# sethdford/csm-mlx

Hardware: AMD Instinct MI355X
Metric: audio frames/sec (24 kHz) csm_1b greedy, 10 s utterances, 1/2/4/8 GPU (higher is better)
Workload: dtype bf16; 1 GPU; csm_1b greedy generate(), 10 s utterances (125 frames) + Mimi decode; top_k=0, stream=False, context_segments=0, model=csm_1b (synthetic seed-0 weights), global_batch=1, per_gpu_batch=1, frames=125, mimi_decode=True, parallelism=dp1

## Files before the change

csm-mlx_amd/csrc/dec_frame.hip:

```cpp
#include <type_traits>

#include "c0_process.h"
#include "csm_kernels.h"
#include "handoff.h"
#include "sampler.h"

namespace {

using namespace handoff;

constexpr int NWG = 256, NT = 512;
constexpr int D = 1024, F = 8192, HQ = 8, HKV = 2, HD = 128, NL = DEC_FRAME_LAYERS, DB = 2048;
constexpr int QKV = (HQ + 2 * HKV) * HD;
constexpr int MAXM = 2;
constexpr int VMAX = 2056;

__device__ __forceinline__ void dot8x2(const u32x4_t w, const float* x0, const float* x1, float& s0, float& s1) {
  const float4 a0 = *reinterpret_cast<const float4*>(x0), b0 = *reinterpret_cast<const float4*>(x0 + 4);
  const float4 a1 = *reinterpret_cast<const float4*>(x1), b1 = *reinterpret_cast<const float4*>(x1 + 4);
  float t;
  t = bf16_lo(w.x); s0 = fmaf(t, a0.x, s0); s1 = fmaf(t, a1.x, s1);
  t = bf16_hi(w.x); s0 = fmaf(t, a0.y, s0); s1 = fmaf(t, a1.y, s1);
  t = bf16_lo(w.y); s0 = fmaf(t, a0.z, s0); s1 = fmaf(t, a1.z, s1);
  t = bf16_hi(w.y); s0 = fmaf(t, a0.w, s0); s1 = fmaf(t, a1.w, s1);
  t = bf16_lo(w.z); s0 = fmaf(t, b0.x, s0); s1 = fmaf(t, b1.x, s1);
  t = bf16_hi(w.z); s0 = fmaf(t, b0.y, s0); s1 = fmaf(t, b1.y, s1);
  t = bf16_lo(w.w); s0 = fmaf(t, b0.z, s0); s1 = fmaf(t, b1.z, s1);
  t = bf16_hi(w.w); s0 = fmaf(t, b0.w, s0); s1 = fmaf(t, b1.w, s1);
}

template <int M>
__device__ __forceinline__ void dotm(const u32x4_t w, const float* x0, const float* x1, float& s0, float& s1) {
  if constexpr (M == 2) {
    dot8x2(w, x0, x1, s0, s1);
  } else {
    const float4 a0 = *reinterpret_cast<const float4*>(x0), b0 = *reinterpret_cast<const float4*>(x0 + 4);
    s0 = fmaf(bf16_lo(w.x), a0.x, s0);
    s0 = fmaf(bf16_hi(w.x), a0.y, s0);
    s0 = fmaf(bf16_lo(w.y), a0.z, s0);
    s0 = fmaf(bf16_hi(w.y), a0.w, s0);
    s0 = fmaf(bf16_lo(w.z), b0.x, s0);
    s0 = fmaf(bf16_hi(w.z), b0.y, s0);
    s0 = fmaf(bf16_lo(w.w), b0.z, s0);
    s0 = fmaf(bf16_hi(w.w), b0.w, s0);
  }
}

__device__ __forceinline__ u32x4_t wload(const bf16_t* p) { return *reinterpret_cast<const u32x4_t*>(p); }

struct Lds {
  float x[MAXM][D];
  float xn[MAXM][DB];
  float qkv[MAXM][QKV];
  float att[MAXM][D];
  float qs[HQ][HD];
  float2 rope[MAXM][HD / 2];
  alignas(16) float hb[MAXM][32];
  float red[4 * MAXM][256];
  float wsum[8][MAXM * 8];
  float sq[8][MAXM];
  union {
    float Ks[HKV][32][HD + 4];
    struct {
      float hq[DB / 32][36];
      float hh[DB / 32];
    } h0;
  };
  float Vs[HKV][32][HD];
  float lg[VMAX];
  int flag;
  alignas(16) float xq[MAXM][D / 32][36];
  float xh[MAXM][D / 32];
  alignas(16) float aq[MAXM][D / 32][36];
  float ah[MAXM][D / 32];
  int c0win[C0_WINDOW_MAX];
  float c0b[16];
};

}

namespace {

constexpr int REP = 4;
constexpr size_t G_X = 0;
constexpr size_t G_QKV = G_X + 2 * REP * rs_of(MAXM * D);
constexpr size_t G_PART = G_QKV + 2 * REP * rs_of(MAXM * QKV);
constexpr size_t G_ARG = G_PART + (size_t)2 * NWG * MAXM * D;
constexpr size_t G_LOG = G_ARG + 2 * REP * rs_of(NWG * 2);
constexpr size_t G_GUM = G_LOG + 2 * REP * rs_of(VMAX);
constexpr size_t G_TOTAL = G_GUM + 2 * REP * rs_of(NWG * 3);

struct Ctx : HandoffCtx<DecFrameArgs, Lds, REP> {
  int ps = 0;
  int code = 0;
  __device__ void mark() {
    if (p.stamps && tid == 0 && ps < 496) p.stamps[(size_t)w * DEC_FRAME_STAMPS + 512 + ps] = __builtin_amdgcn_s_memrealtime();
    ++ps;
  }
  __device__ void stamp() const {
    if (p.stamps && tid == 0 && e < DEC_FRAME_STAMPS) p.stamps[(size_t)w * DEC_FRAME_STAMPS + e] = __builtin_amdgcn_s_memrealtime();
  }
};

constexpr int PROBE_DELAY = 16;
constexpr int DELAY_E1 = PROBE_DELAY, DELAY_E3 = PROBE_DELAY, DELAY_E4 = PROBE_DELAY, DELAY_E5 = 40, DELAY_E6 = PROBE_DELAY;
constexpr int REPOLL = 2;

template <int GPT, int DELAY = PROBE_DELAY, typename F>
__device__ __forceinline__ void poll(Ctx& c, const u64* base, const int (&off)[GPT], const bool (&val)[GPT], F&& use) {
  poll_granules<GPT, DELAY, REPOLL>(base, off, val, c.tag(), [&](unsigned spin) { return spin_fail(c, spin); }, use);
  c.stamp();
}

template <int GPT>
__device__ __forceinline__ void gather(Ctx& c, const u64* buf, int n, float* out) {
  int off[GPT];
  bool val[GPT];
#pragma unroll
  for (int u = 0; u < GPT; ++u) {
    off[u] = c.tid + u * NT;
    val[u] = off[u] < n;
  }
  poll<GPT>(c, buf, off, val, [&](const u64 (&g)[GPT]) {
#pragma unroll
    for (int u = 0; u < GPT; ++u)
      if (val[u]) out[off[u]] = __uint_as_float((unsigned)g[u]);
  });
  __syncthreads();
}

__device__ __forceinline__ float2 nw_fetch(const Ctx& c, const float* nw) { return make_float2(nw[2 * c.tid], nw[2 * c.tid + 1]); }

template <int M>
__device__ __forceinline__ void rms_rows(Ctx& c, float2 nw) {
  static_assert(D == 2 * NT, "a thread scales elements 2 tid and 2 tid + 1 of each row");
  if (c.wave < M) {
    const float* x = c.L.x[c.wave];
    float s = 0.f;
    for (int k = c.lane; k < D; k += 64) s = fmaf(x[k], x[k], s);
    s = wave_sum(s);
    if (c.lane == 0) c.L.wsum[0][c.wave] = s;
  }
  __syncthreads();
  for (int m = 0; m < M; ++m) {
    const float r = rsqrtf(c.L.wsum[0][m] / (float)D + c.p.eps);
    c.L.xn[m][2 * c.tid] = c.L.x[m][2 * c.tid] * r * nw.x;
    c.L.xn[m][2 * c.tid + 1] = c.L.x[m][2 * c.tid + 1] * r * nw.y;
  }
  __syncthreads();
}

template <int M, int DELAY>
__device__ __forceinline__ void gather_x(Ctx& c, const u64* buf, float2 nw) {
  static_assert(D == 2 * NT, "pair tid of row m is elements 2 tid, 2 tid + 1");
  float sq[MAXM];
  int poff[M];
#pragma unroll
  for (int m = 0; m < M; ++m) poff[m] = m * D + 2 * c.tid;
  poll_pairs<M, DELAY, REPOLL>(buf, 0x7fffffff, poff, c.tag(), [&](unsigned spin) { return spin_fail(c, spin); },
                               [&](const u32x4_t (&g)[M]) {
#pragma unroll
    for (int m = 0; m < M; ++m) {
      const float v0 = __uint_as_float(g[m].x), v1 = __uint_as_float(g[m].z);
      *reinterpret_cast<float2*>(&c.L.x[m][2 * c.tid]) = make_float2(v0, v1);
      *reinterpret_cast<float2*>(&c.L.xn[m][2 * c.tid]) = make_float2(v0 * nw.x, v1 * nw.y);
      sq[m] = fmaf(v1, v1, v0 * v0);
    }
  });
  c.stamp();
#pragma unroll
  for (int m = 0; m < M; ++m) {
    const float t = wave_sum(sq[m]);
    if (c.lane == 0) c.L.sq[c.wave][m] = t;
  }
  __syncthreads();
}
__device__ __forceinline__ float row_rs(const Ctx& c, int m) {
  float s = c.L.sq[0][m];
#pragma unroll
  for (int w = 1; w < 8; ++w) s += c.L.sq[w][m];
  return rsqrtf(s / (float)D + c.p.eps);
}

struct WQkv { u32x4_t a, b; };
struct WO { u32x4_t a; };
constexpr int GU_EARLY = 4;
struct WGu { u32x4_t a[8][2]; };
struct WDn { u32x4_t a[2][2][2]; };
struct WHd { u32x4_t a[2]; u32x4_t x[2]; };

__device__ __forceinline__ void load_qkv(Ctx& c, int l, WQkv& r) {
  if (c.wave < 6) {
    const bf16_t* row = c.p.wqkv[l] + (size_t)(6 * c.w) * D;
    const int v = (c.wave * D + 8 * c.lane) * 2;
    r.a = bload(row, v, 0);
    r.b = bload(row, v, 1024);
  }
}
__device__ __forceinline__ void load_o(Ctx& c, int l, WO& r) {
  const bf16_t* row = c.p.wo[l] + (size_t)(4 * c.w) * D;
  r.a = bload(row, ((c.wave >> 1) * D + 8 * ((c.wave & 1) * 64 + c.lane)) * 2, 0);
}
template <int I0, int I1>
__device__ __forceinline__ void load_gu(Ctx& c, int l, WGu& r) {
  const bf16_t* base = c.p.wgu[l] + (size_t)(64 * c.w) * D;
  const int v = (8 * c.wave * D + 8 * c.lane) * 2;
#pragma unroll
  for (int i = I0; i < I1; ++i) {
    r.a[i][0] = bload(base, v, i * D * 2);
    r.a[i][1] = bload(base, v, i * D * 2 + 1024);
  }
}
__device__ __forceinline__ void load_dn(Ctx& c, int l, WDn& r) {
  const bf16_t* base = c.p.wdc[l] + (size_t)(2 * c.w) * D * 16;
  const int v = c.tid * 16 * 2 * 2;
#pragma unroll
  for (int s = 0; s < 2; ++s)
#pragma unroll
    for (int q = 0; q < 2; ++q) {
      const int so = (q * D * 16 + s * 16) * 2;
      r.a[s][q][0] = bload(base, v, so);
      r.a[s][q][1] = bload(base, v, so + 16);
    }
}
__device__ __forceinline__ void load_head(Ctx& c, const bf16_t* W, int K, WHd& r) {
  const bf16_t* base = W + (size_t)(8 * c.w) * K;
  const int v = (c.wave * K + 8 * c.lane) * 2;
  r.a[0] = bload<2>(base, v, 0);
  r.a[1] = bload<2>(base, v, 1024);
  if (c.wave == 0 && c.w < 3) {
    const bf16_t* xr = W + (size_t)(2048 + c.w) * K;
    r.x[0] = bload<2>(xr, 16 * c.lane, 0);
    r.x[1] = bload<2>(xr, 16 * c.lane, 1024);
  }
}

constexpr int RB = D / 2, SBR = D / 64 * 4;
constexpr int RBH = DB / 2, SBRH = DB / 64 * 4;
constexpr int SB_QKV = QKV * RB, SB_O = D * RB, SB_GU = 2 * F * RB, SB_DN = D * F / 2, SB_PROJ = D * RBH;
struct WQkv4 { u32x4_t a; unsigned s; };
struct WO4 { u32x4_t a; unsigned s; };
struct WGu4 { u32x4_t a[4]; unsigned s[4]; };
struct WDn4 { u32x4_t a[2]; unsigned s[2]; };
__device__ __forceinline__ int hrow(const Ctx& c) { return c.lane >> 5; }
__device__ __forceinline__ int hgi(const Ctx& c) { return c.lane & 31; }

__device__ __forceinline__ void load_qkv4(Ctx& c, int l, WQkv4& r) {
  if (c.wave < 3) {
    const char* W = reinterpret_cast<const char*>(c.p.wqkv[l]);
    const int row = 2 * c.wave + hrow(c);
    r.a = bload(W, row * RB + hgi(c) * 16, 6 * c.w * RB);
    r.s = bload4(W, row * SBR + (hgi(c) >> 1) * 4, SB_QKV + 6 * c.w * SBR);
  }
}
__device__ __forceinline__ void load_o4(Ctx& c, int l, WO4& r) {
  if (c.wave < 2) {
    const char* W = reinterpret_cast<const char*>(c.p.wo[l]);
    const int row = 2 * c.wave + hrow(c);
    r.a = bload(W, row * RB + hgi(c) * 16, 4 * c.w * RB);
    r.s = bload4(W, row * SBR + (hgi(c) >> 1) * 4, SB_O + 4 * c.w * SBR);
  }
}
template <int I0, int I1>
__device__ __forceinline__ void load_gu4(Ctx& c, int l, WGu4& r) {
  const char* W = reinterpret_cast<const char*>(c.p.wgu[l]);
  const int row = 8 * c.wave + hrow(c);
#pragma unroll
  for (int i = I0; i < I1; ++i) {
    r.a[i] = bload(W, row * RB + hgi(c) * 16, (64 * c.w + 2 * i) * RB);
    r.s[i] = bload4(W, row * SBR + (hgi(c) >> 1) * 4, SB_GU + (64 * c.w + 2 * i) * SBR);
  }
}
__device__ __forceinline__ void load_dn4(Ctx& c, int l, WDn4& r) {
  const char* W = reinterpret_cast<const char*>(c.p.wdc[l]);
#pragma unroll
  for (int k = 0; k < 2; ++k) {
    r.a[k] = bload(W, (2 * c.tid + k) * 16, c.w * D * 16);
    r.s[k] = bload4(W, (2 * c.tid + k) * 4, SB_DN + (c.w >> 1) * D * 4);
  }
}

__device__ __forceinline__ void half_group_sum16(const Ctx& c, float v, float* out) {
  v = sum16(v);
  if ((c.tid & 15) == 0) out[c.tid >> 4] = v;
}

template <int M, bool SC>
__device__ __forceinline__ void qkv_publish(Ctx& c, int pos0);
template <int M, bool SC>
__device__ __forceinline__ void phase_qkv(Ctx& c, int pos0, const WQkv& W) {
  if (c.wave < 6) {
    float s0 = 0.f, s1 = 0.f;
    dotm<M>(W.a, c.L.xn[0] + 8 * c.lane, c.L.xn[1] + 8 * c.lane, s0, s1);
    dotm<M>(W.b, c.L.xn[0] + 8 * (c.lane + 64), c.L.xn[1] + 8 * (c.lane + 64), s0, s1);
    s0 = wave_sum(s0);
    if constexpr (M == 2) s1 = wave_sum(s1);
    if (c.lane == 0) { c.L.wsum[c.wave][0] = s0; if constexpr (M == 2) c.L.wsum[c.wave][1] = s1; }
  }
  __syncthreads();
  qkv_publish<M, SC>(c, pos0);
}
template <int M, bool SC>
__device__ __forceinline__ void phase_qkv4(Ctx& c, int pos0, const WQkv4& W) {
  if (c.wave < 3) {
#pragma unroll
    for (int m = 0; m < M; ++m) {
      const float2 h = half_sums(q4dot32(W.a, c.L.xq[m][hgi(c)], W.s, c.L.xh[m][hgi(c)]));
      if (c.lane == 0) { c.L.wsum[2 * c.wave][m] = h.x; c.L.wsum[2 * c.wave + 1][m] = h.y; }
    }
  }
  __syncthreads();
  qkv_publish<M, SC>(c, pos0);
}
template <int M, bool SC>
__device__ __forceinline__ void qkv_publish(Ctx& c, int pos0) {
  if (c.tid < 3 * M * REP) {
    const int pr = c.tid / REP, rr = c.tid % REP, m = pr / 3, j = pr % 3, n = 6 * c.w + 2 * j;
    float a = c.L.wsum[2 * j][m], b = c.L.wsum[2 * j + 1][m];
    if (SC) {
      const float rs = row_rs(c, m);
      a *= rs;
      b *= rs;
    }
    if (n < (HQ + HKV) * HD) {
      const int d = n % HD;
      const float2 cs = c.L.rope[m][d / 2];
      const float y0 = a * cs.x - b * cs.y, y1 = b * cs.x + a * cs.y;
      a = y0;
      b = y1;
    }
    c.put(G_QKV, MAXM * QKV, (size_t)m * QKV + n, a, rr);
    c.put(G_QKV, MAXM * QKV, (size_t)m * QKV + n + 1, b, rr);
  }
}

struct KvRegs { u32x4_t k[4], v[4]; };
__device__ __forceinline__ void kv_issue(Ctx& c, int layer, int pos0, KvRegs& r) {
  const int bytes = HKV * c.p.S_cap * HD * 4;
#pragma unroll
  for (int u = 0; u < 4; ++u) {
    const int idx = c.tid + 512 * u, g = idx >> 10, j = (idx >> 5) & 31, q = idx & 31;
    if (j < pos0) {
      const int off = ((g * c.p.S_cap + j) * HD + 4 * q) * 4;
      r.k[u] = sc1_load16(c.p.kc[layer], off, bytes);
      r.v[u] = sc1_load16(c.p.vc[layer], off, bytes);
    }
  }
}
__device__ __forceinline__ void kv_store(Ctx& c, int pos0, const KvRegs& r) {
#pragma unroll
  for (int u = 0; u < 4; ++u) {
    const int idx = c.tid + 512 * u, g = idx >> 10, j = (idx >> 5) & 31, q = idx & 31;
    if (j < pos0) {
      *reinterpret_cast<u32x4_t*>(&c.L.Ks[g][j][4 * q]) = r.k[u];
      *reinterpret_cast<u32x4_t*>(&c.L.Vs[g][j][4 * q]) = r.v[u];
    }
  }
}

__device__ __forceinline__ void qkv_place(Ctx& c, int m, int r, int pos0, float v) {
  if (r < HQ * HD) c.L.qkv[m][r] = v;
  else if (r < (HQ + HKV) * HD) c.L.Ks[(r - HQ * HD) / HD][pos0 + m][r % HD] = v;
  else c.L.Vs[(r - (HQ + HKV) * HD) / HD][pos0 + m][r % HD] = v;
}
template <int M>
__device__ __forceinline__ void gather_qkv(Ctx& c, const u64* buf, int pos0, const KvRegs& kv) {
  constexpr int NP = M * QKV / 2, GPP = (NP + NT - 1) / NT;
  int poff[GPP];
#pragma unroll
  for (int u = 0; u < GPP; ++u) poff[u] = 2 * min(c.tid + u * NT, NP - 1);
  poll_pairs<GPP, DELAY_E1, REPOLL>(buf, 0x7fffffff, poff, c.tag(), [&](unsigned spin) { return spin_fail(c, spin); },
                                    [&](const u32x4_t (&g)[GPP]) {
#pragma unroll
    for (int u = 0; u < GPP; ++u)
      if (c.tid + u * NT < NP) {
        const int i = poff[u];
        qkv_place(c, i / QKV, i % QKV, pos0, __uint_as_float(g[u].x));
        qkv_place(c, (i + 1) / QKV, (i + 1) % QKV, pos0, __uint_as_float(g[u].z));
      }
  });
  c.stamp();
  kv_store(c, pos0, kv);
  __syncthreads();
}

template <int M, bool Q4 = false>
__device__ __forceinline__ void phase_attn(Ctx& c, int pos0, int layer) {
  const int h = c.wave, g = h / (HQ / HKV);
  const float scale = 0.08838834764831845f;
  const int kj = c.lane & 31, hh = c.lane >> 5;
  for (int m = 0; m < M; ++m) {
    const int pos = pos0 + m, n = pos + 1;
    for (int d = c.lane; d < HD; d += 64) c.L.qs[h][d] = c.L.qkv[m][h * HD + d] * scale;
    __builtin_amdgcn_fence(__ATOMIC_RELEASE, "wavefront");
    __builtin_amdgcn_wave_barrier();
    __builtin_amdgcn_fence(__ATOMIC_ACQUIRE, "wavefront");
    float part = 0.f;
    {
      const float4* k4 = reinterpret_cast<const float4*>(c.L.Ks[g][kj] + hh * (HD / 2));
      const float4* q4 = reinterpret_cast<const float4*>(c.L.qs[h] + hh * (HD / 2));
      float d0 = 0.f, d1 = 0.f, d2 = 0.f, d3 = 0.f;
#pragma unroll
      for (int d4 = 0; d4 < HD / 8; ++d4) {
        const float4 a = k4[d4], q = q4[d4];
        d0 = fmaf(q.x, a.x, d0);
        d1 = fmaf(q.y, a.y, d1);
        d2 = fmaf(q.z, a.z, d2);
        d3 = fmaf(q.w, a.w, d3);
      }
      part = (d0 + d1) + (d2 + d3);
    }
    const float other = __shfl_xor(part, 32, 64);
    float s = hh == 0 ? part + other : other + part;
    if (kj >= n) s = -INFINITY;
    const float mx = wave_max(s);
    const float pj = kj < n ? expf(s - mx) : 0.f;
    const float l_run = wave_sum(hh == 0 ? pj : 0.f);
    const int pji = __float_as_int(pj);
    const int kv = c.lane >> 5, dq = c.lane & 31;
    float4 o = make_float4(0.f, 0.f, 0.f, 0.f);
#pragma unroll
    for (int u0 = 0; u0 < 16; u0 += 8) {
      if (u0 < n) {
        float4 vv[8];
#pragma unroll
        for (int u = 0; u < 8; ++u) vv[u] = *reinterpret_cast<const float4*>(&c.L.Vs[g][16 * kv + u0 + u][4 * dq]);
#pragma unroll
        for (int u = 0; u < 8; ++u) {
          const float pa = __int_as_float(__builtin_amdgcn_readlane(pji, u0 + u));
          const float pb = __int_as_float(__builtin_amdgcn_readlane(pji, 16 + u0 + u));
          const float p = kv ? pb : pa;
          if (16 * kv + u0 + u < n) {
            o.x = fmaf(p, vv[u].x, o.x);
            o.y = fmaf(p, vv[u].y, o.y);
            o.z = fmaf(p, vv[u].z, o.z);
            o.w = fmaf(p, vv[u].w, o.w);
          }
        }
      }
    }
    float4 t;
    t.x = __shfl_xor(o.x, 32, 64);
    t.y = __shfl_xor(o.y, 32, 64);
    t.z = __shfl_xor(o.z, 32, 64);
    t.w = __shfl_xor(o.w, 32, 64);
    if constexpr (Q4) {
      const float inv = 1.f / l_run;
      const float4 ov = make_float4((o.x + t.x) * inv, (o.y + t.y) * inv, (o.z + t.z) * inv, (o.w + t.w) * inv);
      if (kv == 0) *reinterpret_cast<float4*>(&c.L.aq[m][0][0] + q4p(h * HD + 4 * dq)) = ov;
      float hs = (ov.x + ov.y) + (ov.z + ov.w);
      hs += __shfl_xor(hs, 1, 64);
      hs += __shfl_xor(hs, 2, 64);
      hs += __shfl_xor(hs, 4, 64);
      if (kv == 0 && (dq & 7) == 0) c.L.ah[m][4 * h + (dq >> 3)] = hs;
    } else if (kv == 0) {
      const float inv = 1.f / l_run;
      *reinterpret_cast<float4*>(&c.L.att[m][h * HD + 4 * dq]) =
          make_float4((o.x + t.x) * inv, (o.y + t.y) * inv, (o.z + t.z) * inv, (o.w + t.w) * inv);
    }
  }
  if (c.tid < M) {
    const int m = c.tid, r = c.w, gg = r / HD, d = r % HD;
    const size_t off = ((size_t)gg * c.p.S_cap + pos0 + m) * HD + d;
    sc1_store_f(c.p.kc[layer] + off, c.L.Ks[gg][pos0 + m][d]);
    sc1_store_f(c.p.vc[layer] + off, c.L.Vs[gg][pos0 + m][d]);
  }
  __syncthreads();
}

template <int M>
__device__ __forceinline__ void phase_o(Ctx& c, const WO& W) {
  {
    const int k = 8 * ((c.wave & 1) * 64 + c.lane);
    float s0 = 0.f, s1 = 0.f;
    dotm<M>(W.a, c.L.att[0] + k, c.L.att[1] + k, s0, s1);
    s0 = wave_sum(s0);
    if constexpr (M == 2) s1 = wave_sum(s1);
    if (c.lane == 0) { c.L.wsum[c.wave][0] = s0; if constexpr (M == 2) c.L.wsum[c.wave][1] = s1; }
  }
  __syncthreads();
  if (c.tid < 4 * M * REP) {
    const int q = c.tid / REP, m = q / 4, r = q % 4, n = 4 * c.w + r;
    const float o = c.L.wsum[2 * r][m] + c.L.wsum[2 * r + 1][m];
    c.put(G_X, MAXM * D, (size_t)m * D + n, c.L.x[m][n] + o, c.tid % REP);
  }
}

template <int M, bool SC>
__device__ __forceinline__ void phase_mlp(Ctx& c, const WGu& G, const WDn& Wd) {
  {
    float s[8][2];
#pragma unroll
    for (int i = 0; i < 8; ++i) {
      s[i][0] = 0.f;
      s[i][1] = 0.f;
      dotm<M>(G.a[i][0], c.L.xn[0] + 8 * c.lane, c.L.xn[1] + 8 * c.lane, s[i][0], s[i][1]);
      dotm<M>(G.a[i][1], c.L.xn[0] + 8 * (c.lane + 64), c.L.xn[1] + 8 * (c.lane + 64), s[i][0], s[i][1]);
    }
#pragma unroll
    for (int m = 0; m < MAXM; ++m) {
      if (m >= M) break;
      float t[8];
#pragma unroll
      for (int i = 0; i < 8; ++i) t[i] = wave_sum(s[i][m]);
      if (c.lane < 4) {
        const float rs = SC ? row_rs(c, m) : 1.f;
        const float gt = rs * (c.lane == 0 ? t[0] : (c.lane == 1 ? t[2] : (c.lane == 2 ? t[4] : t[6])));
        const float up = rs * (c.lane == 0 ? t[1] : (c.lane == 1 ? t[3] : (c.lane == 2 ? t[5] : t[7])));
        c.L.hb[m][4 * c.wave + c.lane] = silu_f(gt) * up;
      }
    }
  }
  if (c.tid < MAXM) asm volatile("s_waitcnt vmcnt(0)" ::: "memory");
  __syncthreads();
  u64* g = c.buf(G_PART, (size_t)NWG * MAXM * D) + (size_t)c.w * MAXM * D;
  float a[2][2];
#pragma unroll
  for (int s = 0; s < 2; ++s) {
    a[s][0] = 0.f;
    a[s][1] = 0.f;
#pragma unroll
    for (int q = 0; q < 2; ++q) {
      dotm<M>(Wd.a[s][q][0], c.L.hb[0] + 16 * q, c.L.hb[1] + 16 * q, a[s][0], a[s][1]);
      dotm<M>(Wd.a[s][q][1], c.L.hb[0] + 16 * q + 8, c.L.hb[1] + 16 * q + 8, a[s][0], a[s][1]);
    }
  }
  const unsigned tg = c.tag();
  const __amdgpu_buffer_rsrc_t rs = __builtin_amdgcn_make_buffer_rsrc(g, 0, 0x7fffffff, 0x00020000);
#pragma unroll
  for (int m = 0; m < M; ++m) {
    const u32x4_t v = {__float_as_uint(a[0][m]), tg, __float_as_uint(a[1][m]), tg};
    __builtin_amdgcn_raw_buffer_store_b128(__builtin_bit_cast(u32x4_t, v), rs, (m * D + 2 * c.tid) * 8, 0, 16);
  }
}

template <int M>
__device__ __forceinline__ void phase_reduce(Ctx& c) {
  const u64* g = c.buf(G_PART, (size_t)NWG * MAXM * D);
  const int v = c.tid >> 1, half = c.tid & 1;
  int off[2 * M];
#pragma unroll
  for (int m = 0; m < M; ++m)
#pragma unroll
    for (int u = 0; u < 2; ++u) off[2 * m + u] = (v * MAXM + m) * D + 4 * c.w + 2 * half + u;
  int poff[M];
#pragma unroll
  for (int m = 0; m < M; ++m) poff[m] = off[2 * m];
  poll_pairs<M, DELAY_E4, REPOLL>(g, 0x7fffffff, poff, c.tag(), [&](unsigned spin) { return spin_fail(c, spin); },
                                  [&](const u32x4_t (&q)[M]) {
#pragma unroll
    for (int m = 0; m < M; ++m) {
      c.L.red[4 * m + 2 * half][v] = __uint_as_float(q[m].x);
      c.L.red[4 * m + 2 * half + 1][v] = __uint_as_float(q[m].z);
    }
  });
  c.stamp();
  __syncthreads();
  ++c.e;
  if (c.wave < 4 * M) {
    const float* r = c.L.red[c.wave];
    float s = ((r[4 * c.lane] + r[4 * c.lane + 1]) + r[4 * c.lane + 2]) + r[4 * c.lane + 3];
    s = wave_sum(s);
    if (c.lane < REP) {
      const int m = c.wave / 4, n = 4 * c.w + c.wave % 4;
      c.put(G_X, MAXM * D, (size_t)m * D + n, c.L.x[m][n] + s, c.lane);
    }
  }
}

template <int M>
__device__ __forceinline__ void phase_o4(Ctx& c, const WO4& W) {
  if (c.wave < 2) {
#pragma unroll
    for (int m = 0; m < M; ++m) {
      const float2 h = half_sums(q4dot32(W.a, c.L.aq[m][hgi(c)], W.s, c.L.ah[m][hgi(c)]));
      if (c.lane == 0) { c.L.wsum[2 * c.wave][m] = h.x; c.L.wsum[2 * c.wave + 1][m] = h.y; }
    }
  }
  __syncthreads();
  if (c.tid < 4 * M * REP) {
    const int q = c.tid / REP, m = q / 4, r = q % 4, n = 4 * c.w + r;
    c.put(G_X, MAXM * D, (size_t)m * D + n, c.L.x[m][n] + c.L.wsum[r][m], c.tid % REP);
  }
}
template <int M, bool SC>
__device__ __forceinline__ void phase_mlp4(Ctx& c, const WGu4& G, const WDn4& Wd) {
#pragma unroll
  for (int m = 0; m < M; ++m) {
    const float rs = SC ? row_rs(c, m) : 1.f;
#pragma unroll
    for (int i = 0; i < 4; ++i) {
      const float2 h = half_sums(q4dot32(G.a[i], c.L.xq[m][hgi(c)], G.s[i], c.L.xh[m][hgi(c)]));
      if (c.lane == i) c.L.hb[m][4 * c.wave + i] = silu_f(rs * h.x) * (rs * h.y);
    }
  }
  if (c.tid < MAXM) asm volatile("s_waitcnt vmcnt(0)" ::: "memory");
  __syncthreads();
  u64* g = c.buf(G_PART, (size_t)NWG * MAXM * D) + (size_t)c.w * MAXM * D;
  const unsigned tg = c.tag();
  const __amdgpu_buffer_rsrc_t rsc = __builtin_amdgcn_make_buffer_rsrc(g, 0, 0x7fffffff, 0x00020000);
#pragma unroll
  for (int m = 0; m < M; ++m) {
    float hs = 0.f;
#pragma unroll
    for (int j = 0; j < 32; j += 4) {
      const float4 v = *reinterpret_cast<const float4*>(&c.L.hb[m][j]);
      hs += (v.x + v.y) + (v.z + v.w);
    }
    const float a0 = q4dot32(Wd.a[0], c.L.hb[m], Wd.s[0], hs), a1 = q4dot32(Wd.a[1], c.L.hb[m], Wd.s[1], hs);
    const u32x4_t v = {__float_as_uint(a0), tg, __float_as_uint(a1), tg};
    __builtin_amdgcn_raw_buffer_store_b128(__builtin_bit_cast(u32x4_t, v), rsc, (m * D + 2 * c.tid) * 8, 0, 16);
  }
}
template <int M, int DELAY>
__device__ __forceinline__ void gather_x4(Ctx& c, const u64* buf, float2 nw) {
  int poff[M];
#pragma unroll
  for (int m = 0; m < M; ++m) poff[m] = m * D + 2 * c.tid;
  float sq[MAXM], pr[MAXM];
  poll_pairs<M, DELAY, REPOLL>(buf, 0x7fffffff, poff, c.tag(), [&](unsigned spin) { return spin_fail(c, spin); },
                               [&](const u32x4_t (&g)[M]) {
#pragma unroll
    for (int m = 0; m < M; ++m) {
      const float v0 = __uint_as_float(g[m].x), v1 = __uint_as_float(g[m].z);
      const float a = v0 * nw.x, b = v1 * nw.y;
      *reinterpret_cast<float2*>(&c.L.x[m][2 * c.tid]) = make_float2(v0, v1);
      *reinterpret_cast<float2*>(&c.L.xq[m][0][0] + q4p(2 * c.tid)) = make_float2(a, b);
      sq[m] = fmaf(v1, v1, v0 * v0);
      pr[m] = a + b;
    }
  });
  c.stamp();
#pragma unroll
  for (int m = 0; m < M; ++m) {
    half_group_sum16(c, pr[m], c.L.xh[m]);
    const float t = wave_sum(sq[m]);
    if (c.lane == 0) c.L.sq[c.wave][m] = t;
  }
  __syncthreads();
}
template <int M>
__device__ __forceinline__ void rms_rows4(Ctx& c, float2 nw) {
  if (c.wave < M) {
    const float* x = c.L.x[c.wave];
    float s = 0.f;
    for (int k = c.lane; k < D; k += 64) s = fmaf(x[k], x[k], s);
    s = wave_sum(s);
    if (c.lane == 0) c.L.wsum[0][c.wave] = s;
  }
  __syncthreads();
#pragma unroll
  for (int m = 0; m < M; ++m) {
    const float r = rsqrtf(c.L.wsum[0][m] / (float)D + c.p.eps);
    const float a = c.L.x[m][2 * c.tid] * r * nw.x, b = c.L.x[m][2 * c.tid + 1] * r * nw.y;
    *reinterpret_cast<float2*>(&c.L.xq[m][0][0] + q4p(2 * c.tid)) = make_float2(a, b);
    half_group_sum16(c, a + b, c.L.xh[m]);
  }
  __syncthreads();
}

__device__ __forceinline__ bool gumbel_local(const DecFrameArgs& p) {
  return p.temperature > 0.f && (p.top_k <= 0 || p.top_k >= p.V);
}
__device__ __forceinline__ unsigned long long dkey(double d) {
  const unsigned long long u = (unsigned long long)__double_as_longlong(d);
  return (u >> 63) ? ~u : (u | (1ull << 63));
}

template <bool C0 = false>
__device__ __forceinline__ void head_publish(Ctx& c, float s, float t, int n_valid, float* logits, int cb);
template <int KH, bool PAD = false, bool C0 = false>
__device__ __forceinline__ void phase_head(Ctx& c, const bf16_t* W, int n_valid, const u32x4_t (&wa)[KH / 512],
                                           const u32x4_t (&wx)[KH / 512], float* logits, int cb, int xm = 0, float rs = 1.f) {
  constexpr int CPL = KH / 512;
  static_assert(!PAD || KH == D, "the padded input holds one decoder row");
  auto xin = [&](int i) -> const float* {
    if constexpr (PAD) return &c.L.xq[xm][0][0] + q4p(8 * (c.lane + 64 * i));
    else return c.L.xn[xm] + 8 * (c.lane + 64 * i);
  };
  float s = 0.f;
#pragma unroll
  for (int i = 0; i < CPL; ++i) s += dot8(wa[i], xin(i));
  s = wave_sum(s) * rs;
  float t = 0.f;
  if (c.wave == 0 && c.w < 3) {
#pragma unroll
    for (int i = 0; i < CPL; ++i) t += dot8(wx[i], xin(i));
    t = wave_sum(t) * rs;
  }
  head_publish<C0>(c, s, t, n_valid, logits, cb);
  (void)W;
}
template <bool C0>
__device__ __forceinline__ void head_publish(Ctx& c, float s, float t, int n_valid, float* logits, int cb) {
  const int row = 8 * c.w + c.wave;
  if constexpr (C0) {
    if (c.p.c0_bias || c.p.c0_penalty > 0.f) {
      const int n = c0_window_n(c.p.frame_ctr[0], c.p.c0_context, c.p.c0_penalty);
      s = c0_processed(s, row, c.p.c0_bias, c.L.c0b[c.wave], c.L.c0win, n, c.p.c0_penalty);
      if (c.wave == 0 && c.w < 3) t = c0_processed(t, 2048 + c.w, c.p.c0_bias, c.L.c0b[8], c.L.c0win, n, c.p.c0_penalty);
    }
  }
  unsigned long long best = row < n_valid ? pack_argmax(s, row) : 0ull;
  if (c.lane == 0 && row < n_valid) logits[row] = s;
  const int xr = 2048 + c.w;
  if (c.wave == 0 && c.w < 3) {
    const unsigned long long k2 = xr < n_valid ? pack_argmax(t, xr) : 0ull;
    best = k2 > best ? k2 : best;
    if (c.lane == 0 && xr < n_valid) logits[xr] = t;
  }
  if (gumbel_local(c.p)) {
    const float inv_t = 1.0f / c.p.temperature;
    const uint64_t key = gumbel_key(c.p.seeds[0], c.p.frame_ctr[0] * c.p.K + cb);
    unsigned long long bk = 0ull;
    int bi = 0x7fffffff;
    auto cand = [&](float l, int v) {
      if (!(l >= -INFINITY)) return;
      double val = (double)(l * inv_t) + gumbel_noise(key, v);
      if (!(val > -INFINITY)) return;
      if (val == 0.0) val = 0.0;
      const unsigned long long k = dkey(val);
      if (k > bk || (k == bk && v < bi)) { bk = k; bi = v; }
    };
    if (c.lane == 0 && row < n_valid) cand(s, row);
    if (c.lane == 0 && c.wave == 0 && c.w < 3 && xr < n_valid) cand(t, xr);
    unsigned long long* gk = reinterpret_cast<unsigned long long*>(&c.L.wsum[0][0]);
    int* gi = reinterpret_cast<int*>(gk + 8);
    if (c.lane == 0) { gk[c.wave] = bk; gi[c.wave] = bi; }
    __syncthreads();
    if (c.tid < REP) {
      unsigned long long b = gk[0];
      int ib = gi[0];
      for (int i = 1; i < 8; ++i)
        if (gk[i] > b || (gk[i] == b && gi[i] < ib)) { b = gk[i]; ib = gi[i]; }
      c.put_u(G_GUM, NWG * 3, 3 * c.w, (unsigned)(b >> 32), c.tid);
      c.put_u(G_GUM, NWG * 3, 3 * c.w + 1, (unsigned)b, c.tid);
      c.put_u(G_GUM, NWG * 3, 3 * c.w + 2, (unsigned)ib, c.tid);
    }
    __syncthreads();
    return;
  }
  if (c.p.temperature > 0.f) {
    if (c.lane < REP && row < n_valid) c.put(G_LOG, VMAX, row, s, c.lane);
    if (c.lane < REP && c.wave == 0 && c.w < 3 && xr < n_valid) c.put(G_LOG, VMAX, xr, t, c.lane);
    __syncthreads();
    return;
  }
  if (c.lane == 0) reinterpret_cast<unsigned long long*>(c.L.wsum)[c.wave] = best;
  __syncthreads();
  if (c.tid < REP) {
    const unsigned long long* k = reinterpret_cast<const unsigned long long*>(c.L.wsum);
    unsigned long long b = k[0];
    for (int i = 1; i < 8; ++i) b = k[i] > b ? k[i] : b;
    c.put_u(G_ARG, NWG * 2, 2 * c.w, (unsigned)(b >> 32), c.tid);
    c.put_u(G_ARG, NWG * 2, 2 * c.w + 1, (unsigned)b, c.tid);
  }
  __syncthreads();
}

__device__ __forceinline__ int gather_code(Ctx& c, int V) {
  static_assert(NWG <= NT, "one key per thread");
  unsigned long long b = 0ull;
  if (c.tid < NWG) {
    const int poff[1] = {2 * c.tid};
    poll_pairs<1, DELAY_E6, REPOLL>(c.rbuf(G_ARG, NWG * 2), 0x7fffffff, poff, c.tag(),
                                    [&](unsigned spin) { return spin_fail(c, spin); },
                                    [&](const u32x4_t (&g)[1]) { b = ((unsigned long long)g[0].x << 32) | g[0].z; });
  }
  c.stamp();
#pragma unroll
  for (int o = 32; o > 0; o >>= 1) {
    const unsigned long long t = __shfl_xor(b, o, 64);
    b = t > b ? t : b;
  }
  unsigned long long* wk = reinterpret_cast<unsigned long long*>(&c.L.red[0][0]);
  if (c.lane == 0) wk[c.wave] = b;
  __syncthreads();
  b = wk[0];
#pragma unroll
  for (int i = 1; i < NT / 64; ++i) b = wk[i] > b ? wk[i] : b;
  c.code = min(max(unpack_argmax(b), 0), V - 1);
  return c.code;
}

__device__ __forceinline__ int sample_code(Ctx& c, int V, int cb) {
  constexpr int NPT = sampler::DEC_FRAME_SAMPLE_NPT;
  static_assert(VMAX <= NT * NPT, "a slot for every logit");
  static_assert(sizeof(sampler::Scratch<NT / 64>) <= sizeof(Lds::red), "the sampler borrows L.red");
  const DecFrameArgs& p = c.p;
  const uint64_t key = gumbel_key(p.seeds[0], p.frame_ctr[0] * p.K + cb);
  double gn[NPT];
#pragma unroll
  for (int i = 0; i < NPT; ++i) {
    const int v = c.tid + NT * i;
    gn[i] = v < V ? gumbel_noise(key, v) : 0.0;
  }
  gather<NPT>(c, c.rbuf(G_LOG, VMAX), V, c.L.lg);
  sampler::Scratch<NT / 64>& S = *reinterpret_cast<sampler::Scratch<NT / 64>*>(&c.L.red[0][0]);
  auto logit = [&](int i) { return c.L.lg[c.tid + NT * i]; };
  float thr = -INFINITY;
  if (p.top_k > 0 && p.top_k < V) thr = sampler::topk_threshold<NT, NPT>(c.tid, V, p.top_k, S.hist, S.wsum, S.sh, logit);
  double best;
  int bi;
  sampler::gumbel_pass<NT, NPT>(c.tid, V, thr, 1.0f / p.temperature, logit, [&](int i, int) { return gn[i]; }, best, bi);
  c.code = sampler::clamp_code(sampler::block_argmax<double, NT / 64>(c.tid, best, bi, S.bv, S.bi), V);
  __syncthreads();
  return c.code;
}

__device__ __forceinline__ int gumbel_code(Ctx& c, int V) {
  constexpr int NG = NWG * 3, GPT = (NG + NT - 1) / NT;
  int off[GPT];
  bool val[GPT];
#pragma unroll
  for (int u = 0; u < GPT; ++u) {
    off[u] = c.tid + u * NT;
    val[u] = off[u] < NG;
  }
  unsigned* words = reinterpret_cast<unsigned*>(&c.L.red[0][0]);
  poll<GPT, DELAY_E6>(c, c.rbuf(G_GUM, NWG * 3), off, val, [&](const u64 (&g)[GPT]) {
#pragma unroll
    for (int u = 0; u < GPT; ++u)
      if (val[u]) words[off[u]] = (unsigned)g[u];
  });
  __syncthreads();
  unsigned long long b = 0ull;
  int ib = 0x7fffffff;
  if (c.tid < NWG) {
    b = ((unsigned long long)words[3 * c.tid] << 32) | words[3 * c.tid + 1];
    ib = (int)words[3 * c.tid + 2];
  }
#pragma unroll
  for (int o = 32; o > 0; o >>= 1) {
    const unsigned long long ob = __shfl_xor(b, o, 64);
    const int oi = __shfl_xor(ib, o, 64);
    if (ob > b || (ob == b && oi < ib)) { b = ob; ib = oi; }
  }
  unsigned long long* wk = reinterpret_cast<unsigned long long*>(&c.L.wsum[0][0]);
  int* wi = reinterpret_cast<int*>(wk + 8);
  __syncthreads();
  if (c.lane == 0 && c.wave < NWG / 64) { wk[c.wave] = b; wi[c.wave] = ib; }
  __syncthreads();
  b = wk[0];
  ib = wi[0];
#pragma unroll
  for (int i = 1; i < NWG / 64; ++i)
    if (wk[i] > b || (wk[i] == b && wi[i] < ib)) { b = wk[i]; ib = wi[i]; }
  c.code = b == 0ull ? V - 1 : min(max(ib, 0), V - 1);
  return c.code;
}

__device__ __forceinline__ int head_code(Ctx& c, int V, int cb) {
  if (c.p.temperature <= 0.f) return gather_code(c, V);
  return gumbel_local(c.p) ? gumbel_code(c, V) : sample_code(c, V, cb);
}

struct Pre {
  WQkv wq;
  WO wo;
  WGu wg;
  WDn wd;
  WHd wh;
  float2 nw1;
};
struct Pre4 {
  WQkv4 wq;
  WO4 wo;
  WGu4 wg;
  WDn4 wd;
  WHd wh;
  float2 nw1;
};
template <bool Q4> using PreT = std::conditional_t<Q4, Pre4, Pre>;
constexpr int GU4_EARLY = 2;
template <bool Q4, typename P> __device__ __forceinline__ void ld_dn(Ctx& c, int l, P& r) {
  if constexpr (Q4) load_dn4(c, l, r.wd); else load_dn(c, l, r.wd);
}
template <bool Q4, typename P> __device__ __forceinline__ void ld_qkv(Ctx& c, int l, P& r) {
  if constexpr (Q4) load_qkv4(c, l, r.wq); else load_qkv(c, l, r.wq);
}
template <bool Q4, typename P> __device__ __forceinline__ void ld_o(Ctx& c, int l, P& r) {
  if constexpr (Q4) load_o4(c, l, r.wo); else load_o(c, l, r.wo);
}
template <bool Q4, bool EARLY, typename P> __device__ __forceinline__ void ld_gu(Ctx& c, int l, P& r) {
  if constexpr (Q4) {
    if constexpr (EARLY) load_gu4<0, GU4_EARLY>(c, l, r.wg); else load_gu4<GU4_EARLY, 4>(c, l, r.wg);
  } else {
    if constexpr (EARLY) load_gu<0, GU_EARLY>(c, l, r.wg); else load_gu<GU_EARLY, 8>(c, l, r.wg);
  }
}

template <int M, bool FIRST, bool LAST, bool Q4>
__device__ __forceinline__ void decoder_layer(Ctx& c, int l, int step, int pos0, PreT<Q4>& r) {
  const DecFrameArgs& p = c.p;
  Lds& L = c.L;
  c.refresh();
  float2 rp = make_float2(0.f, 0.f);
  if (FIRST && c.tid < M * (HD / 2))
    rp = reinterpret_cast<const float2*>(p.rope)[(size_t)pos0 * (HD / 2) + c.tid];
  if (FIRST && step > 1) {
    const float* t = p.qkv0_tab + ((size_t)(step - 1) * p.V + c.code) * QKV;
    const float* xr = p.proj_tab + ((size_t)(step - 1) * p.V + c.code) * D;
    constexpr int NQ4 = QKV / 4, NX4 = D / 4;
    const float4* t4 = reinterpret_cast<const float4*>(t);
    const float4* x4 = reinterpret_cast<const float4*>(xr);
    const int i0 = c.tid, i1 = NT + c.tid;
    const float4 va = i0 < NQ4 ? t4[i0] : x4[i0 - NQ4];
    const float4 vb = i1 < NQ4 + NX4 ? x4[min(i1, NQ4 + NX4 - 1) - NQ4] : make_float4(0.f, 0.f, 0.f, 0.f);
    ld_dn<Q4>(c, l, r);
    auto put4 = [&](int i, const float4 v) {
      if (i < NQ4) {
        qkv_place(c, 0, 4 * i, pos0, v.x);
        qkv_place(c, 0, 4 * i + 1, pos0, v.y);
        qkv_place(c, 0, 4 * i + 2, pos0, v.z);
        qkv_place(c, 0, 4 * i + 3, pos0, v.w);
      } else {
        *reinterpret_cast<float4*>(&L.x[0][4 * (i - NQ4)]) = v;
      }
    };
    put4(i0, va);
    if (i1 < NQ4 + NX4) put4(i1, vb);
    if (c.tid < M * (HD / 2)) L.rope[c.tid / (HD / 2)][c.tid % (HD / 2)] = rp;
    __syncthreads();
  } else {
    KvRegs kv;
    if (FIRST && c.tid < M * (HD / 2)) L.rope[c.tid / (HD / 2)][c.tid % (HD / 2)] = rp;
    if constexpr (Q4) {
      if (FIRST) rms_rows4<M>(c, r.nw1);
      phase_qkv4<M, !FIRST>(c, pos0, r.wq);
    } else {
      if (FIRST) rms_rows<M>(c, r.nw1);
      phase_qkv<M, !FIRST>(c, pos0, r.wq);
    }
    kv_issue(c, l, pos0, kv);
    ld_dn<Q4>(c, l, r);
    gather_qkv<M>(c, c.rbuf(G_QKV, MAXM * QKV), pos0, kv);
    ++c.e;
  }
  c.refresh();
  c.mark();
  const float2 nw2 = nw_fetch(c, p.n2[l]);
  ld_gu<Q4, true>(c, l, r);
  phase_attn<M, Q4>(c, pos0, l);
  c.mark();
  if constexpr (Q4) phase_o4<M>(c, r.wo);
  else phase_o<M>(c, r.wo);
  c.mark();
  ld_gu<Q4, false>(c, l, r);
  if (!LAST) { ld_qkv<Q4>(c, l + 1, r); ld_o<Q4>(c, l + 1, r); }
  if constexpr (Q4) gather_x4<M, DELAY_E3>(c, c.rbuf(G_X, MAXM * D), nw2);
  else gather_x<M, DELAY_E3>(c, c.rbuf(G_X, MAXM * D), nw2);
  ++c.e;
  c.refresh();
  if constexpr (Q4) phase_mlp4<M, true>(c, r.wg, r.wd);
  else phase_mlp<M, true>(c, r.wg, r.wd);
  r.nw1 = nw_fetch(c, LAST ? p.norm : p.n1[l + 1]);
  c.mark();
  if (LAST) {
    load_head(c, p.audio_head + (size_t)(step - 1) * p.VP * D, D, r.wh);
    if (step + 1 < p.K) {
      ld_o<Q4>(c, 0, r);
      ld_qkv<Q4>(c, 1, r);
    }
  }
  c.refresh();
  phase_reduce<M>(c);
  if constexpr (Q4) gather_x4<M, DELAY_E5>(c, c.rbuf(G_X, MAXM * D), r.nw1);
  else gather_x<M, DELAY_E5>(c, c.rbuf(G_X, MAXM * D), r.nw1);
  ++c.e;
}

template <int M, bool Q4>
__device__ __forceinline__ void run_step(Ctx& c, int step, PreT<Q4>& r) {
  const DecFrameArgs& p = c.p;
  const int pos0 = M == 2 ? 0 : step;
  decoder_layer<M, true, false, Q4>(c, 0, step, pos0, r);
  for (int l = 1; l < NL - 1; ++l) decoder_layer<M, false, false, Q4>(c, l, step, pos0, r);
  decoder_layer<M, false, true, Q4>(c, NL - 1, step, pos0, r);
  c.refresh();
  phase_head<D, Q4>(c, p.audio_head + (size_t)(step - 1) * p.VP * D, p.V, r.wh.a, r.wh.x, p.ci_logits + (size_t)(step - 1) * p.VP,
                    step, M - 1, row_rs(c, M - 1));
  KvRegs kv0;
  if (step + 1 < p.K) kv_issue(c, 0, step + 1, kv0);
  const int ci = head_code(c, p.V, step);
  ++c.e;
  if (c.w == 0 && c.tid == 0) p.codes[step] = ci;
  if (step + 1 < p.K) kv_store(c, step + 1, kv0);
}

__device__ __forceinline__ void c0_stage(Ctx& c) {
  const DecFrameArgs& p = c.p;
  if (p.c0_bias && c.tid < 9) {
    const int v = c.tid < 8 ? 8 * c.w + c.tid : 2048 + c.w;
    c.L.c0b[c.tid] = v < p.VP ? p.c0_bias[v] : 0.f;
  }
  if (p.c0_penalty > 0.f) {
    const int f = p.frame_ctr[0];
    if (c.tid < c0_window_n(f, p.c0_context, p.c0_penalty)) c.L.c0win[c.tid] = c0_window_code(p.hist, f, c.tid, 0, 1, p.K);
  }
}

__device__ __forceinline__ void frame_start4(Ctx& c) {
  const DecFrameArgs& p = c.p;
  Lds& L = c.L;
  const char* H = reinterpret_cast<const char*>(p.c0_head);
  const char* P = reinterpret_cast<const char*>(p.proj);
  const int sbh = p.VP * RBH;
  const u32x4_t ha = bload(H, c.wave * RBH + c.lane * 16, 8 * c.w * RBH);
  const unsigned hs = bload4(H, c.wave * SBRH + (c.lane >> 1) * 4, sbh + 8 * c.w * SBRH);
  u32x4_t hx = {0u, 0u, 0u, 0u};
  unsigned hxs = 0u;
  if (c.wave == 0 && c.w < 3) {
    hx = bload(H, c.lane * 16, (2048 + c.w) * RBH);
    hxs = bload4(H, (c.lane >> 1) * 4, sbh + (2048 + c.w) * SBRH);
  }
  const int pw = min(c.wave, 3);
  const u32x4_t pa = bload(P, pw * RBH + c.lane * 16, 4 * c.w * RBH);
  const unsigned ps = bload4(P, pw * SBRH + (c.lane >> 1) * 4, SB_PROJ + 4 * c.w * SBRH);
#pragma unroll
  for (int h = 0; h < 2; ++h) {
    const int k = h * (DB / 2) + 2 * c.tid;
    const float2 v = *reinterpret_cast<const float2*>(p.h_last + k);
    *reinterpret_cast<float2*>(&L.h0.hq[0][0] + q4p(k)) = v;
    float sum = v.x + v.y;
    sum += __shfl_xor(sum, 1, 64);
    sum += __shfl_xor(sum, 2, 64);
    sum += __shfl_xor(sum, 4, 64);
    sum += __shfl_xor(sum, 8, 64);
    if ((c.tid & 15) == 0) L.h0.hh[k >> 5] = sum;
  }
  c0_stage(c);
  __syncthreads();
  const float s = wave_sum(q4dot32(ha, L.h0.hq[c.lane], hs, L.h0.hh[c.lane]));
  float t = 0.f;
  if (c.wave == 0 && c.w < 3) t = wave_sum(q4dot32(hx, L.h0.hq[c.lane], hxs, L.h0.hh[c.lane]));
  head_publish<true>(c, s, t, p.V, p.c0_logits, 0);
  const float pv = wave_sum(q4dot32(pa, L.h0.hq[c.lane], ps, L.h0.hh[c.lane]));
  if (c.lane == 0 && c.wave < 4) L.wsum[c.wave][0] = pv;
  __syncthreads();
  if (c.tid < 4 * REP) {
    const int q = c.tid / REP;
    c.put(G_X, MAXM * D, 4 * c.w + q, L.wsum[q][0], c.tid % REP);
  }
}
}

template <bool Q4>
__global__ __launch_bounds__(NT, 1) void dec_frame_kernel(DecFrameArgs p) {
  __shared__ __attribute__((aligned(16))) Lds L;
  Ctx c{{p, L, (int)blockIdx.x, (int)threadIdx.x, (int)(threadIdx.x & 63), (int)(threadIdx.x >> 6), 0u, 0}};
  c.tag0 = __hip_atomic_load(p.epoch, __ATOMIC_RELAXED, __HIP_MEMORY_SCOPE_AGENT) + 1u;
  if (p.stamps && c.tid == 0) p.stamps[(size_t)c.w * DEC_FRAME_STAMPS + DEC_FRAME_STAMPS - 2] = __builtin_amdgcn_s_memrealtime();
  PreT<Q4> r;
  if constexpr (Q4) {
    ld_qkv<Q4>(c, 0, r);
    ld_o<Q4>(c, 0, r);
    frame_start4(c);
  } else {
  u32x4_t c0a[4], c0x[4], pa[2];
  {
    const bf16_t* row = p.c0_head + (size_t)(8 * c.w) * DB;
#pragma unroll
    for (int i = 0; i < 4; ++i) c0a[i] = bload(row, (c.wave * DB + 8 * c.lane) * 2, i * 1024);
    if (c.wave == 0 && c.w < 3) {
      const bf16_t* xr = p.c0_head + (size_t)(2048 + c.w) * DB;
#pragma unroll
      for (int i = 0; i < 4; ++i) c0x[i] = bload(xr, 16 * c.lane, i * 1024);
    }
    const bf16_t* pr = p.proj + (size_t)(4 * c.w) * DB;
    const int pv = ((c.wave >> 1) * DB + 8 * 128 * (c.wave & 1) + 8 * c.lane) * 2;
    pa[0] = bload(pr, pv, 0);
    pa[1] = bload(pr, pv, 1024);
  }
  load_qkv(c, 0, r.wq);
  load_o(c, 0, r.wo);
  for (int k = c.tid; k < DB; k += NT) L.xn[0][k] = p.h_last[k];
  c0_stage(c);
  __syncthreads();
  phase_head<DB, false, true>(c, p.c0_head, p.V, c0a, c0x, p.c0_logits, 0);
  {
    float s = dot8(pa[0], L.xn[0] + 8 * (128 * (c.wave & 1) + c.lane)) + dot8(pa[1], L.xn[0] + 8 * (128 * (c.wave & 1) + c.lane + 64));
    s = wave_sum(s);
    if (c.lane == 0) L.wsum[c.wave][0] = s;
    __syncthreads();
    if (c.tid < 4 * REP) {
      const int q = c.tid / REP;
      c.put(G_X, MAXM * D, 4 * c.w + q, L.wsum[2 * q][0] + L.wsum[2 * q + 1][0], c.tid % REP);
    }
  }
  }
  const int c0 = head_code(c, p.V, 0);
  gather<2>(c, c.rbuf(G_X, MAXM * D), D, L.x[0]);
  ++c.e;
  if (c.w == 0 && c.tid == 0) p.codes[0] = c0;
  for (int k = c.tid; k < D; k += NT) L.x[1][k] = p.proj_tab[(size_t)c0 * D + k];
  __syncthreads();

  r.nw1 = nw_fetch(c, p.n1[0]);
  run_step<2, Q4>(c, 1, r);
  for (int step = 2; step < p.K; ++step) run_step<1, Q4>(c, step, r);
  if (p.stamps && c.tid == 0) p.stamps[(size_t)c.w * DEC_FRAME_STAMPS + DEC_FRAME_STAMPS - 1] = __builtin_amdgcn_s_memrealtime();
  if (c.w == 0 && c.tid == 0) __hip_atomic_store(p.epoch, c.tag0 - 1u + (unsigned)c.e, __ATOMIC_RELAXED, __HIP_MEMORY_SCOPE_AGENT);
}

size_t dec_frame_gbuf_bytes() { return G_TOTAL * sizeof(u64); }

void launch_dec_frame(const DecFrameArgs& p, hipStream_t st, bool q4) {
  if (q4) hipLaunchKernelGGL(dec_frame_kernel<true>, dim3(NWG), dim3(NT), 0, st, p);
  else hipLaunchKernelGGL(dec_frame_kernel<false>, dim3(NWG), dim3(NT), 0, st, p);
}

const void* dec_frame_kernel_ptr(bool q4) {
  return q4 ? reinterpret_cast<const void*>(&dec_frame_kernel<true>) : reinterpret_cast<const void*>(&dec_frame_kernel<false>);
}
```

Baseline: 419.5 audio frames/s.

## Streamline decoder attention with pre-scaled Q, DPP/permlane swaps, and guarded PV

Q values are scaled by the attention scale when gathered into LDS. This drops the per-wave copy into a separate qs buffer and the wave barrier and fences that went with it. The PV accumulation is rearranged so that each lane pair covers 16-lane groups: probabilities are broadcast with DPP row moves instead of readlane, and the half-wave reductions use permlane32/permlane16 swaps instead of shfl_xor. V in LDS is zeroed at kernel start so that unguarded rows contribute zero, and the KV-cache writeback is moved ahead of the attention loop to overlap it. The risks are correctness of the new lane mapping and reliance on gfx950-specific permlane intrinsics.

New measurement: 421.4 audio frames/s (median of 6 runs). Within noise of the previous version (+0.4%).

```diff
diff --git a/csm-mlx_amd/csrc/dec_frame.hip b/csm-mlx_amd/csrc/dec_frame.hip
--- a/csm-mlx_amd/csrc/dec_frame.hip
+++ b/csm-mlx_amd/csrc/dec_frame.hip
@@ -14,6 +14,7 @@
 constexpr int QKV = (HQ + 2 * HKV) * HD;
 constexpr int MAXM = 2;
 constexpr int VMAX = 2056;
+constexpr float ATTN_SCALE = 0.08838834764831845f;
 
 __device__ __forceinline__ void dot8x2(const u32x4_t w, const float* x0, const float* x1, float& s0, float& s1) {
   const float4 a0 = *reinterpret_cast<const float4*>(x0), b0 = *reinterpret_cast<const float4*>(x0 + 4);
@@ -51,9 +52,8 @@
 struct Lds {
   float x[MAXM][D];
   float xn[MAXM][DB];
-  float qkv[MAXM][QKV];
+  float qs[MAXM][HQ * HD];
   float att[MAXM][D];
-  float qs[HQ][HD];
   float2 rope[MAXM][HD / 2];
   alignas(16) float hb[MAXM][32];
   float red[4 * MAXM][256];
@@ -359,7 +359,7 @@
 }
 
 __device__ __forceinline__ void qkv_place(Ctx& c, int m, int r, int pos0, float v) {
-  if (r < HQ * HD) c.L.qkv[m][r] = v;
+  if (r < HQ * HD) c.L.qs[m][r] = v * ATTN_SCALE;
   else if (r < (HQ + HKV) * HD) c.L.Ks[(r - HQ * HD) / HD][pos0 + m][r % HD] = v;
   else c.L.Vs[(r - (HQ + HKV) * HD) / HD][pos0 + m][r % HD] = v;
 }
@@ -384,21 +384,45 @@
   __syncthreads();
 }
 
+template <int U, bool GUARD>
+__device__ __forceinline__ void pv_key(float4& o, int pji, const float4 v, int nk) {
+  const float p = __int_as_float(__builtin_amdgcn_mov_dpp(pji, 0x150 + U, 0xF, 0xF, true));
+  if (!GUARD || U < nk) {
+    o.x = fmaf(p, v.x, o.x);
+    o.y = fmaf(p, v.y, o.y);
+    o.z = fmaf(p, v.z, o.z);
+    o.w = fmaf(p, v.w, o.w);
+  }
+}
+template <int U0>
+__device__ __forceinline__ void pv_load(float4 (&vv)[16], const float* v) {
+#pragma unroll
+  for (int u = U0; u < U0 + 4; ++u) vv[u] = *reinterpret_cast<const float4*>(v + u * HD);
+}
+template <int U0, bool GUARD>
+__device__ __forceinline__ void pv_rows(float4& o, int pji, const float4 (&vv)[16], int nk) {
+  pv_key<U0, GUARD>(o, pji, vv[U0], nk);
+  pv_key<U0 + 1, GUARD>(o, pji, vv[U0 + 1], nk);
+  pv_key<U0 + 2, GUARD>(o, pji, vv[U0 + 2], nk);
+  pv_key<U0 + 3, GUARD>(o, pji, vv[U0 + 3], nk);
+}
 template <int M, bool Q4 = false>
 __device__ __forceinline__ void phase_attn(Ctx& c, int pos0, int layer) {
+  if (c.tid < M) {
+    const int m = c.tid, r = c.w, gg = r / HD, d = r % HD;
+    const size_t off = ((size_t)gg * c.p.S_cap + pos0 + m) * HD + d;
+    sc1_store_f(c.p.kc[layer] + off, c.L.Ks[gg][pos0 + m][d]);
+    sc1_store_f(c.p.vc[layer] + off, c.L.Vs[gg][pos0 + m][d]);
+  }
   const int h = c.wave, g = h / (HQ / HKV);
-  const float scale = 0.08838834764831845f;
   const int kj = c.lane & 31, hh = c.lane >> 5;
+  const int kv = (c.lane >> 4) & 1, dq = (c.lane & 15) | ((c.lane >> 5) << 4);
   for (int m = 0; m < M; ++m) {
     const int pos = pos0 + m, n = pos + 1;
-    for (int d = c.lane; d < HD; d += 64) c.L.qs[h][d] = c.L.qkv[m][h * HD + d] * scale;
-    __builtin_amdgcn_fence(__ATOMIC_RELEASE, "wavefront");
-    __builtin_amdgcn_wave_barrier();
-    __builtin_amdgcn_fence(__ATOMIC_ACQUIRE, "wavefront");
     float part = 0.f;
     {
       const float4* k4 = reinterpret_cast<const float4*>(c.L.Ks[g][kj] + hh * (HD / 2));
-      const float4* q4 = reinterpret_cast<const float4*>(c.L.qs[h] + hh * (HD / 2));
+      const float4* q4 = reinterpret_cast<const float4*>(c.L.qs[m] + h * HD + hh * (HD / 2));
       float d0 = 0.f, d1 = 0.f, d2 = 0.f, d3 = 0.f;
 #pragma unroll
       for (int d4 = 0; d4 < HD / 8; ++d4) {
@@ -410,43 +434,38 @@
       }
       part = (d0 + d1) + (d2 + d3);
     }
-    const float other = __shfl_xor(part, 32, 64);
-    float s = hh == 0 ? part + other : other + part;
+    const auto ph = __builtin_amdgcn_permlane32_swap(__float_as_uint(part), __float_as_uint(part), false, false);
+    float s = __uint_as_float(ph[0]) + __uint_as_float(ph[1]);
     if (kj >= n) s = -INFINITY;
     const float mx = wave_max(s);
     const float pj = kj < n ? expf(s - mx) : 0.f;
     const float l_run = wave_sum(hh == 0 ? pj : 0.f);
     const int pji = __float_as_int(pj);
-    const int kv = c.lane >> 5, dq = c.lane & 31;
     float4 o = make_float4(0.f, 0.f, 0.f, 0.f);
-#pragma unroll
-    for (int u0 = 0; u0 < 16; u0 += 8) {
-      if (u0 < n) {
-        float4 vv[8];
-#pragma unroll
-        for (int u = 0; u < 8; ++u) vv[u] = *reinterpret_cast<const float4*>(&c.L.Vs[g][16 * kv + u0 + u][4 * dq]);
-#pragma unroll
-        for (int u = 0; u < 8; ++u) {
-          const float pa = __int_as_float(__builtin_amdgcn_readlane(pji, u0 + u));
-          const float pb = __int_as_float(__builtin_amdgcn_readlane(pji, 16 + u0 + u));
-          const float p = kv ? pb : pa;
-          if (16 * kv + u0 + u < n) {
-            o.x = fmaf(p, vv[u].x, o.x);
-            o.y = fmaf(p, vv[u].y, o.y);
-            o.z = fmaf(p, vv[u].z, o.z);
-            o.w = fmaf(p, vv[u].w, o.w);
-          }
-        }
-      }
-    }
-    float4 t;
-    t.x = __shfl_xor(o.x, 32, 64);
-    t.y = __shfl_xor(o.y, 32, 64);
-    t.z = __shfl_xor(o.z, 32, 64);
-    t.w = __shfl_xor(o.w, 32, 64);
+    {
+      const float* v = &c.L.Vs[g][16 * kv][4 * dq];
+      const int nk = n - 16 * kv;
+      float4 vv[16];
+      pv_load<0>(vv, v);
+      if (4 < n) pv_load<4>(vv, v);
+      if (8 < n) pv_load<8>(vv, v);
+      if (12 < n) pv_load<12>(vv, v);
+      pv_rows<0, M == 2>(o, pji, vv, nk);
+      if (4 < n) pv_rows<4, M == 2>(o, pji, vv, nk);
+      if (8 < n) pv_rows<8, M == 2>(o, pji, vv, nk);
+      if (12 < n) pv_rows<12, M == 2>(o, pji, vv, nk);
+    }
+    float4 ov;
+    {
+      const auto tx = __builtin_amdgcn_permlane16_swap(__float_as_uint(o.x), __float_as_uint(o.x), false, false);
+      const auto ty = __builtin_amdgcn_permlane16_swap(__float_as_uint(o.y), __float_as_uint(o.y), false, false);
+      const auto tz = __builtin_amdgcn_permlane16_swap(__float_as_uint(o.z), __float_as_uint(o.z), false, false);
+      const auto tw = __builtin_amdgcn_permlane16_swap(__float_as_uint(o.w), __float_as_uint(o.w), false, false);
+      const float inv = 1.f / l_run;
+      ov = make_float4((__uint_as_float(tx[0]) + __uint_as_float(tx[1])) * inv, (__uint_as_float(ty[0]) + __uint_as_float(ty[1])) * inv,
+                       (__uint_as_float(tz[0]) + __uint_as_float(tz[1])) * inv, (__uint_as_float(tw[0]) + __uint_as_float(tw[1])) * inv);
+    }
     if constexpr (Q4) {
-      const float inv = 1.f / l_run;
-      const float4 ov = make_float4((o.x + t.x) * inv, (o.y + t.y) * inv, (o.z + t.z) * inv, (o.w + t.w) * inv);
       if (kv == 0) *reinterpret_cast<float4*>(&c.L.aq[m][0][0] + q4p(h * HD + 4 * dq)) = ov;
       float hs = (ov.x + ov.y) + (ov.z + ov.w);
       hs += __shfl_xor(hs, 1, 64);
@@ -454,16 +473,8 @@
       hs += __shfl_xor(hs, 4, 64);
       if (kv == 0 && (dq & 7) == 0) c.L.ah[m][4 * h + (dq >> 3)] = hs;
     } else if (kv == 0) {
-      const float inv = 1.f / l_run;
-      *reinterpret_cast<float4*>(&c.L.att[m][h * HD + 4 * dq]) =
-          make_float4((o.x + t.x) * inv, (o.y + t.y) * inv, (o.z + t.z) * inv, (o.w + t.w) * inv);
-    }
-  }
-  if (c.tid < M) {
-    const int m = c.tid, r = c.w, gg = r / HD, d = r % HD;
-    const size_t off = ((size_t)gg * c.p.S_cap + pos0 + m) * HD + d;
-    sc1_store_f(c.p.kc[layer] + off, c.L.Ks[gg][pos0 + m][d]);
-    sc1_store_f(c.p.vc[layer] + off, c.L.Vs[gg][pos0 + m][d]);
+      *reinterpret_cast<float4*>(&c.L.att[m][h * HD + 4 * dq]) = ov;
+    }
   }
   __syncthreads();
 }
@@ -1051,6 +1062,7 @@
   Ctx c{{p, L, (int)blockIdx.x, (int)threadIdx.x, (int)(threadIdx.x & 63), (int)(threadIdx.x >> 6), 0u, 0}};
   c.tag0 = __hip_atomic_load(p.epoch, __ATOMIC_RELAXED, __HIP_MEMORY_SCOPE_AGENT) + 1u;
   if (p.stamps && c.tid == 0) p.stamps[(size_t)c.w * DEC_FRAME_STAMPS + DEC_FRAME_STAMPS - 2] = __builtin_amdgcn_s_memrealtime();
+  for (int i = c.tid; i < HKV * 32 * HD / 4; i += NT) reinterpret_cast<float4*>(&L.Vs[0][0][0])[i] = make_float4(0.f, 0.f, 0.f, 0.f);
   PreT<Q4> r;
   if constexpr (Q4) {
     ld_qkv<Q4>(c, 0, r);
```
